# syghmon/bridges-with-reinforcement-learning

Hardware: AMD Instinct MI355X
Metric: env-steps/sec (vectorised assembly_gym, tower_height=4) (higher is better)
Workload: dtype f64

## Files before the change

bridges-with-reinforcement-learning_amd/bridges_hip/abi.py:

```python
import ctypes as C
import os

HERE = os.path.dirname(os.path.abspath(__file__))
LIB_PATH = os.environ.get("BRIDGES_LIB", os.path.join(HERE, "libbridges_hip.so"))
CSRC_DIR = os.path.join(os.path.dirname(HERE), "csrc")
INCLUDE_DIR = os.path.join(os.path.dirname(os.path.dirname(HERE)), "include")
STAMP_PREFIX = "BRIDGES_SRC_HASH="


def source_hash():
    import hashlib
    h = hashlib.sha256()
    for tag, d in (("csrc", CSRC_DIR), ("include", INCLUDE_DIR)):
        for name in sorted(os.listdir(d)):
            path = os.path.join(d, name)
            if os.path.isfile(path) and not name.startswith("."):
                h.update(f"{tag}/{name}\0".encode())
                with open(path, "rb") as fh:
                    h.update(fh.read())
                h.update(b"\0")
    return h.hexdigest()


def library_stamp(path=None):
# ... 127 lines not shown
def lib():
    global _lib
    if _lib is not None:
        return _lib
    if not os.path.exists(LIB_PATH):
        raise BridgesHipError(
            f"{LIB_PATH} not found: build it with `python __graft_entry__.py build` "
            "(hipcc --offload-arch=gfx950).  There is no CPU fallback.")
    L = C.CDLL(LIB_PATH)
    vp, i32, i64, f64, f32 = C.c_void_p, C.c_int32, C.c_int64, C.c_double, C.c_float
    try:
        L.bridges_source_hash.restype = C.c_char_p
        stamp = L.bridges_source_hash().decode()[len(STAMP_PREFIX):]
    except AttributeError:
        stamp = "missing"
    want = source_hash()
    if stamp != want:
        raise BridgesHipError(f"{LIB_PATH} is stale: it was built from other sources (stamp {stamp[:16]}, sources {want[:16]}); "
                              "rebuild it with `python __graft_entry__.py build`")
    L.bridges_last_error.restype = C.c_char_p
    L.bridges_device_count.restype = C.c_int
    sigs = {
        "bridges_env_create": [C.POINTER(Task), C.POINTER(EnvBuffers), C.POINTER(vp)],
        "bridges_env_destroy": [vp],
        "bridges_env_reset": [vp, vp],
        "bridges_env_step": [vp, vp],
        "bridges_env_select_random": [vp, vp],
        "bridges_env_lockstep_random": [vp, vp],
        "bridges_env_refresh": [vp, vp],
        "bridges_env_candidate_stability": [vp, vp],
        "bridges_gate_create": [C.POINTER(vp)],
        "bridges_gate_destroy": [vp],
        "bridges_env_set_gate": [vp, vp],
        "bridges_env_timing_begin": [vp, i32],
        "bridges_env_timing_end": [vp, C.POINTER(C.c_double), C.POINTER(i32)],
        "bridges_shapes_upload": [C.POINTER(Shape), i32, C.POINTER(vp)],
        "bridges_shapes_free": [vp],
        "bridges_place": [vp, i32, vp, vp, vp, vp, vp, vp, vp, vp],
        "bridges_create_block": [vp, i32, vp, vp, vp, vp, vp, vp, vp, vp, vp, vp, vp],
        "bridges_pose_block": [vp, i32, vp, vp, vp, vp],
        "bridges_face_frames": [vp, i32, vp, vp, vp, vp],
        "bridges_contains_points": [vp, i32, vp, i32, vp, vp, vp],
        "bridges_raster": [vp, i32, vp, vp, vp, vp, vp, vp, vp],
        "bridges_raster_sized": [vp, i32, vp, vp, vp, vp, i32, vp, vp, vp],
        "bridges_render_blocks": [vp, i32, vp, vp, vp, i32, vp, i32, vp, vp],
        "bridges_bits_or": [i32, vp, vp, vp, vp],
        "bridges_action_features": [vp, i32, vp, vp, vp, vp, i32, f64, f64, f64, f64, vp, vp, vp, vp, vp, vp, vp, vp],
        "bridges_bits_to_f32": [i32, vp, vp, vp],
        "bridges_bits_linear": [i32, vp, vp, vp, i32, vp, vp, vp, vp],
        "bridges_sigmoid_dot": [i32, vp, i64, vp, i32, vp, vp],
        "bridges_bits_dot": [i32, vp, vp, vp, vp, vp, vp],
        "bridges_head_sigmoid_dot": [i32, i32, i32, vp, i64, vp, vp, vp, vp, vp, i32, vp],
        "bridges_linear_backward_log": [i32, i32, i32, vp, vp, vp, vp, vp, vp, vp, vp, i64, vp, i32, vp, i32, vp, vp, vp],
        "bridges_mlp_mid_rows": [i32, i32, vp, vp, vp, vp, i64, vp, i64, vp, vp],
        "bridges_mlp_mid_supported": [i32, i32, vp],
        "bridges_mlp_mid_forward": [i32, i32, vp, vp, vp, vp, vp],
        "bridges_mlp_mid_backward": [i32, i32, vp, vp, vp, vp, vp, vp, vp, vp, vp, vp, i64, vp, f64, f64, f64, f64, vp],
        "bridges_eps_greedy_select": [i32, i32, vp, vp, vp, vp, vp, C.c_float, i32, vp, vp, vp, vp, vp, vp, vp, vp],
        "bridges_valid_rows": [i32, vp, vp, vp, vp, vp, vp, vp, vp, vp, vp, vp, vp],
        "bridges_env_groups": [i32, i32, vp, vp, vp, vp, vp, vp, vp, vp],
        "bridges_record_state": [i32, i32, vp, vp, vp, vp, vp, vp, vp, vp, vp, vp],
        "bridges_record_result": [i32, vp, vp, vp, vp, vp, vp],
        "bridges_replay_unpack": [i32, i32, i32, vp, vp, i32, i32, i32, i32, vp, vp, vp, vp, vp, vp, vp, vp, vp, vp, vp, vp],
        "bridges_bits_accumulate": [i32, vp, vp, vp, vp, vp, vp],
        "bridges_stability": [vp, i32, i32, vp, vp, vp, vp, vp, f64, f64, f64, f64, vp, vp, vp, i64, vp],
        "bridges_stability_penalty": [vp, i32, i32, vp, vp, vp, vp, vp, f64, f64, f64, f64, f64, vp, vp, vp, vp, i64, vp],
# ... 6 lines not shown
        "bridges_linear_forward": [i32, i32, i32, vp, vp, vp, i32, vp, vp, i64, vp, vp],
        "bridges_linear_backward": [i32, i32, i32, vp, vp, vp, vp, vp, vp, vp, vp, i64, vp, i32, vp],
        "bridges_mlp_input": [i32, i32, i32, i32, vp, vp, vp, vp, vp, vp, vp, vp],
        "bridges_mlp_input_batches": [i32, i32, i32, i32, i32, vp, vp, vp, vp, vp, vp, vp],
        "bridges_successor_loss": [i32, i32, i32, i32, vp, vp, vp, vp, vp, i32, i32, vp, vp, vp, vp, i32, vp, vp, vp, vp],
        "bridges_adam_step": [vp, vp, vp, vp, i64, vp, f64, f64, f64, f64, vp],
        "bridges_linear_backward_adam": [i32, i32, i32, vp, vp, vp, vp, vp, vp, vp, vp, vp, vp, vp, vp, i64, vp, f64, f64, f64, f64, vp, i32, vp],
        "bridges_conv3x3": [vp, vp, vp, vp, vp, vp, i64, i32, i32, i32, i32, i32, vp],
        "bridges_conv3x3_wgrad_scratch": [i64, i32, i32, i32, C.POINTER(i64)],
        "bridges_conv3x3_wgrad": [vp, vp, vp, vp, vp, vp, i64, i64, i32, i32, i32, vp],
        "bridges_maxpool2": [vp, vp, i64, i32, i32, vp],
        "bridges_bias_grad": [vp, vp, vp, i64, i64, i32, i32, vp],
        "bridges_adam_multi": [vp, i32, vp, vp, i32, vp, f64, f64, f64, f64, vp],
        "bridges_reduce_jobs": [vp, i32, i32, vp],
        "bridges_upconv2x2_backward_scratch": [i64, i32, i32, i32, i32, C.POINTER(i64)],
        "bridges_upconv2x2_backward": [vp, vp, vp, vp, vp, vp, vp, i64, i64, i32, i32, i32, i32, vp],
        "bridges_conv1x1_o1_forward": [vp, vp, vp, vp, i64, i32, i32, vp],
        "bridges_conv1x1_o1_backward": [vp, vp, vp, vp, vp, vp, vp, i64, i64, i32, i32, vp],
        "bridges_maxpool2_relu_backward": [vp, vp, vp, i64, i32, i32, vp],
        "bridges_td_target": [i32, vp, vp, vp, vp, i64, vp, vp, vp, f32, i32, vp, vp, vp, vp],
    }
    for name, argtypes in sigs.items():
        fn = getattr(L, name)
        fn.argtypes = argtypes
        fn.restype = C.c_int
    _lib = L
    return L


EXPORTED_SYMBOLS = (
    "bridges_last_error", "bridges_device_count", "bridges_source_hash", "bridges_env_create", "bridges_env_destroy",
    "bridges_env_reset", "bridges_env_step", "bridges_env_select_random", "bridges_env_lockstep_random", "bridges_env_refresh",
    "bridges_env_candidate_stability",
    "bridges_gate_create", "bridges_gate_destroy", "bridges_env_set_gate",
    "bridges_env_timing_begin", "bridges_env_timing_end",
    "bridges_place", "bridges_create_block", "bridges_pose_block", "bridges_face_frames", "bridges_contains_points", "bridges_raster", "bridges_raster_sized", "bridges_render_blocks", "bridges_action_features", "bridges_bits_or", "bridges_bits_to_f32", "bridges_bits_linear", "bridges_bits_dot", "bridges_bits_accumulate", "bridges_head_sigmoid_dot", "bridges_linear_backward_log", "bridges_mlp_mid_rows", "bridges_mlp_mid_supported", "bridges_mlp_mid_forward", "bridges_mlp_mid_backward", "bridges_eps_greedy_select", "bridges_valid_rows", "bridges_env_groups", "bridges_record_state", "bridges_record_result", "bridges_replay_unpack", "bridges_sigmoid_dot", "bridges_stability", "bridges_stability_penalty",
    "bridges_shapes_upload", "bridges_shapes_free", "bridges_soft_update", "bridges_td_target", "bridges_bias_relu", "bridges_bias_relu_pool2",
    "bridges_conv3x3_relu_o16", "bridges_conv3x3_relu_o16_ex", "bridges_conv3x3", "bridges_conv3x3_wgrad_scratch", "bridges_conv3x3_wgrad",
    "bridges_maxpool2", "bridges_maxpool2_relu_backward", "bridges_bias_grad", "bridges_adam_multi", "bridges_reduce_jobs", "bridges_upconv2x2_backward_scratch", "bridges_upconv2x2_backward", "bridges_conv1x1_o1_forward", "bridges_conv1x1_o1_backward", "bridges_upconv2x2", "bridges_linear_forward", "bridges_linear_backward", "bridges_mlp_input", "bridges_mlp_input_batches", "bridges_successor_loss", "bridges_adam_step", "bridges_linear_backward_adam",
)


def check(rc, what=""):
    if rc != 0:
        msg = lib().bridges_last_error().decode(errors="replace")
        raise BridgesHipError(f"{what} failed (rc={rc}): {msg}")


def require_gpu():
    import torch
    L = lib()
    if not torch.cuda.is_available() or L.bridges_device_count() <= 0:
        raise BridgesHipError("no MI355X / HIP device visible: the assembly_gym hot path runs only on the "
                              "HIP kernels of libbridges_hip.so (no CPU fallback)")
    return L


def current_stream():
    import torch
    return C.c_void_p(torch._C._cuda_getCurrentRawStream(torch._C._cuda_getDevice()))
```

bridges-with-reinforcement-learning_amd/csrc/api.hip:

```cpp
#include <hip/hip_runtime.h>
#include <cstdio>
#include <cstdlib>
#include <cstring>
#include <new>

#include "env_kernels.hip"
#include "ops_kernels.hip"
#include "dqn_kernels.hip"
#include "mlp_kernels.hip"
#include "conv_kernels.hip"
#include "conv_train_kernels.hip"

using namespace bridges;

static thread_local char g_err[512] = "";

static int fail_hip(hipError_t e, const char* what) {
    snprintf(g_err, sizeof(g_err), "%s: %s", what, hipGetErrorString(e));
    return BRIDGES_E_HIP;
}
static int fail_arg(const char* what) {
    snprintf(g_err, sizeof(g_err), "bad argument: %s", what);
    return BRIDGES_E_ARG;
}
#define HIP_TRY(x)                                        \
    do {                                                  \
        hipError_t e_ = (x);                              \
        if (e_ != hipSuccess) return fail_hip(e_, #x);    \
    } while (0)
#define LAUNCH_CHECK(name)                                       \
    do {                                                         \
        hipError_t e_ = hipGetLastError();                       \
        if (e_ != hipSuccess) return fail_hip(e_, name);         \
    } while (0)

struct bridges_gate {
    hipEvent_t last;
};

struct bridges_env {
    bridges_gate* gate;
    hipEvent_t raster_done;
    DevCtx ctx;
    TaskTable* tt_dev;
    int32_t* h_total;
    int max_blocks;
    int max_faces;
    hipEvent_t* ev_start;
    hipEvent_t* ev_stop;
    int ev_cap, ev_used;
};

extern "C" {

const char* bridges_last_error(void) { return g_err; }

#ifndef BRIDGES_SRC_HASH
#define BRIDGES_SRC_HASH "unstamped"
#endif
const char* bridges_source_hash(void) { return "BRIDGES_SRC_HASH=" BRIDGES_SRC_HASH; }

int bridges_device_count(void) {
    int n = 0;
    if (hipGetDeviceCount(&n) != hipSuccess) return 0;
    return n;
}

int bridges_env_create(const bridges_task* t, const bridges_env_buffers* buf, bridges_env** out) {
    if (!t || !buf || !out) return fail_arg("null");
    if (t->n_envs <= 0) return fail_arg("n_envs");
    if (t->max_blocks <= 0 || t->max_blocks > BRIDGES_MAX_BLOCKS) return fail_arg("max_blocks > BRIDGES_MAX_BLOCKS");
    if (t->n_shapes <= 0 || t->n_shapes > 8) return fail_arg("n_shapes");
    if (t->n_groups <= 0 || t->n_groups > BRIDGES_MAX_GROUPS) return fail_arg("n_groups");
    if (t->n_ground < 0 || t->n_ground > 32 || t->n_offsets <= 0 || t->n_offsets > 8) return fail_arg("n_ground/n_offsets");
    if (t->n_targets < 0 || t->n_targets > BRIDGES_MAX_TARGETS) return fail_arg("n_targets");
// ... 28 lines not shown
    memcpy(host->offsets, t->offsets, sizeof(double) * t->n_offsets);
    const int img = t->img_size ? t->img_size : IMG;
    for (int i = 0; i < IMG; ++i) {
        host->grid_x[i] = t->grid_x[i < img ? i : img - 1];
        host->grid_y[i] = t->grid_y[i < img ? i : img - 1];
    }
    hipError_t e = hipMalloc((void**)&env->tt_dev, sizeof(TaskTable));
    if (e == hipSuccess) e = hipMemcpy(env->tt_dev, host, sizeof(TaskTable), hipMemcpyHostToDevice);
    delete host;
    if (e != hipSuccess) { delete env; return fail_hip(e, "task table upload"); }
    DevCtx& c = env->ctx;
    memset(&c, 0, sizeof(c));
    c.b = *buf;
    c.tt = env->tt_dev;
    c.E = t->n_envs; c.K = t->max_blocks; c.max_steps = t->max_steps; c.a_max = t->a_max;
    c.n_groups = t->n_groups; c.n_ground = t->n_ground; c.n_offsets = t->n_offsets; c.n_targets = t->n_targets;
    memcpy(c.group_shape, t->group_shape, sizeof(c.group_shape));
    memcpy(c.group_face, t->group_face, sizeof(c.group_face));
    c.mu = t->mu; c.density = t->density; c.floor_hw = t->floor_half_width; c.floor_depth = t->floor_depth;
    c.xlim0 = t->xlim[0]; c.xlim1 = t->xlim[1]; c.ylim0 = t->ylim[0]; c.ylim1 = t->ylim[1];
    memcpy(c.targets, t->targets, sizeof(c.targets));
    c.seed = t->seed;
    c.debug = t->debug;
    c.env_id_base = t->env_id_base;
    c.n_shapes = t->n_shapes;
    c.img = img;
    hipDeviceProp_t prop;
    int dev = 0;
    (void)hipGetDevice(&dev);
    env->ev_start = env->ev_stop = nullptr;
    env->ev_cap = env->ev_used = 0;
    env->gate = nullptr;
    env->raster_done = nullptr;
    int cus = 256;
    if (hipGetDeviceProperties(&prop, dev) == hipSuccess && prop.multiProcessorCount > 0) cus = prop.multiProcessorCount;
    (void)cus;
    e = hipHostMalloc((void**)&env->h_total, sizeof(int32_t), hipHostMallocMapped | hipHostMallocCoherent);
    if (e == hipSuccess) e = hipHostGetDevicePointer((void**)&c.h_total, env->h_total, 0);
    if (e != hipSuccess) { (void)hipFree(env->tt_dev); delete env; return fail_hip(e, "hipHostMalloc"); }
    *env->h_total = t->n_envs * 64;
    env->max_blocks = 1 << 22;
    env->max_faces = 0;
    for (int g = 0; g < t->n_groups; ++g) {
        const int nv = t->shapes[t->group_shape[g]].nv;
        if (nv > env->max_faces) env->max_faces = nv;
    }
    *out = env;
    return BRIDGES_OK;
}

static void free_events(bridges_env* env) {
    for (int i = 0; i < env->ev_cap; ++i) {
        (void)hipEventDestroy(env->ev_start[i]);
        (void)hipEventDestroy(env->ev_stop[i]);
    }
    delete[] env->ev_start;
    delete[] env->ev_stop;
    env->ev_start = env->ev_stop = nullptr;
    env->ev_cap = env->ev_used = 0;
}

int bridges_env_destroy(bridges_env* env) {
    if (!env) return BRIDGES_OK;
    free_events(env);
    if (env->raster_done) (void)hipEventDestroy(env->raster_done);
    (void)hipFree(env->tt_dev);
    (void)hipHostFree(env->h_total);
    delete env;
    return BRIDGES_OK;
}

int bridges_gate_create(bridges_gate** out) {
    if (!out) return fail_arg("gate_create");
    bridges_gate* g = new (std::nothrow) bridges_gate();
    if (!g) return fail_arg("oom");
    g->last = nullptr;
    *out = g;
    return BRIDGES_OK;
}

int bridges_gate_destroy(bridges_gate* gate) {
    delete gate;
    return BRIDGES_OK;
}

int bridges_env_set_gate(bridges_env* env, bridges_gate* gate) {
    if (!env) return fail_arg("set_gate");
    if (gate && !env->raster_done) HIP_TRY(hipEventCreateWithFlags(&env->raster_done, hipEventDisableTiming));
    env->gate = gate;
    return BRIDGES_OK;
}

int bridges_env_timing_begin(bridges_env* env, int32_t max_launches) {
    if (!env || max_launches <= 0 || max_launches > (1 << 16)) return fail_arg("timing_begin");
    free_events(env);
    env->ev_start = new (std::nothrow) hipEvent_t[max_launches];
    env->ev_stop = new (std::nothrow) hipEvent_t[max_launches];
    if (!env->ev_start || !env->ev_stop) {
        delete[] env->ev_start;
        delete[] env->ev_stop;
        env->ev_start = env->ev_stop = nullptr;
        return fail_arg("oom");
    }
    for (int i = 0; i < max_launches; ++i) {
        HIP_TRY(hipEventCreate(&env->ev_start[i]));
        HIP_TRY(hipEventCreate(&env->ev_stop[i]));
        env->ev_cap = i + 1;
    }
    env->ev_used = 0;
    return BRIDGES_OK;
}

int bridges_env_timing_end(bridges_env* env, double* raster_ms_total, int32_t* n_launches) {
    if (!env || !raster_ms_total || !n_launches) return fail_arg("timing_end");
    double total = 0.0;
    for (int i = 0; i < env->ev_used; ++i) {
        HIP_TRY(hipEventSynchronize(env->ev_stop[i]));
        float ms = 0.f;
        HIP_TRY(hipEventElapsedTime(&ms, env->ev_start[i], env->ev_stop[i]));
        total += ms;
    }
    *raster_ms_total = total;
    *n_launches = env->ev_used;
    free_events(env);
    return BRIDGES_OK;
}

#ifndef RASTER_DYN_LDS
#define RASTER_DYN_LDS 0
#endif
static int refresh(bridges_env* env, hipStream_t s, int after_step) {
    const DevCtx& c = env->ctx;
    hipLaunchKernelGGL(k_scan, dim3(1), dim3(SCAN_THREADS), 0, s, c, after_step);
    LAUNCH_CHECK("k_scan");
    hipLaunchKernelGGL(k_enumerate, dim3(c.E), dim3(WAVE), 0, s, c);
    LAUNCH_CHECK("k_enumerate");
    long long est = (long long)(*(volatile int32_t*)env->h_total);
    if (est < c.E) est = c.E;
    est += est / 32 + 64;
    const long long items_est = est + c.E;
    long long rblocks = (items_est + 3) / 4;
    if (rblocks > env->max_blocks) rblocks = env->max_blocks;
    const bool timed = env->ev_cap > 0 && env->ev_used < env->ev_cap;
    if (env->gate && env->gate->last) HIP_TRY(hipStreamWaitEvent(s, env->gate->last, 0));
    if (timed) HIP_TRY(hipEventRecord(env->ev_start[env->ev_used], s));
    if (env->max_faces <= 4) hipLaunchKernelGGL(k_raster<4>, dim3((unsigned)rblocks), dim3(256), RASTER_DYN_LDS, s, c);
    else hipLaunchKernelGGL(k_raster<MAXV>, dim3((unsigned)rblocks), dim3(256), RASTER_DYN_LDS, s, c);
    LAUNCH_CHECK("k_raster");
    if (timed) { HIP_TRY(hipEventRecord(env->ev_stop[env->ev_used], s)); env->ev_used++; }
    if (env->gate) {
        HIP_TRY(hipEventRecord(env->raster_done, s));
        env->gate->last = env->raster_done;
    }
    hipLaunchKernelGGL(k_select, dim3(c.E), dim3(WAVE), 0, s, c, 0);
    LAUNCH_CHECK("k_select");
    return BRIDGES_OK;
}

int bridges_env_reset(bridges_env* env, void* stream) {
    if (!env) return fail_arg("null env");
    hipStream_t s = (hipStream_t)stream;
    hipLaunchKernelGGL(k_reset, dim3(env->ctx.E), dim3(WAVE), 0, s, env->ctx);
    LAUNCH_CHECK("k_reset");
    return refresh(env, s, 0);
}

int bridges_env_step(bridges_env* env, void* stream) {
    if (!env) return fail_arg("null env");
    hipStream_t s = (hipStream_t)stream;
    hipLaunchKernelGGL(k_step, dim3(env->ctx.E), dim3(WAVE), 0, s, env->ctx);
    LAUNCH_CHECK("k_step");
    return refresh(env, s, 1);
}

int bridges_env_refresh(bridges_env* env, void* stream) {
    if (!env) return fail_arg("null env");
    return refresh(env, (hipStream_t)stream, 0);
}

#ifndef CS_TAB_SMALL
#define CS_TAB_SMALL 768
#endif
#ifndef CS_COLS_SMALL
#define CS_COLS_SMALL 92
#endif
#define CS_TAB_LARGE 4096
int bridges_env_candidate_stability(bridges_env* env, void* stream) {
    if (!env) return fail_arg("null env");
    const DevCtx& c = env->ctx;
    if (!c.b.cand_stable || !c.b.cand_queue || !c.b.cand_counters || !c.b.cand_ws) return fail_arg("cand_stable / cand_queue / cand_counters / cand_ws not given");
    if (c.b.cand_ws_stride < (int64_t)(3 * c.K + 2) * (4 * BRIDGES_MAX_INTERFACES + 3)) return fail_arg("cand_ws_stride");
    hipStream_t s = (hipStream_t)stream;
    HIP_TRY(hipMemsetAsync(c.b.cand_counters, 0, 2 * sizeof(int32_t), s));
    long long est = (long long)(*(volatile int32_t*)env->h_total);
    if (est < c.E) est = c.E;
    est += est / 32 + 64;
    if (est > env->max_blocks) est = env->max_blocks;
    hipLaunchKernelGGL((k_candidate_stability<CS_TAB_SMALL, CS_COLS_SMALL, false>), dim3((unsigned)est), dim3(WAVE), 0, s, c);
    LAUNCH_CHECK("k_candidate_stability");
    const int drain = BRIDGES_CAND_WS_SLOTS;
    hipLaunchKernelGGL((k_candidate_stability<CS_TAB_LARGE, LP_MAX_COLS, true>), dim3(drain), dim3(WAVE), 0, s, c);
    LAUNCH_CHECK("k_candidate_stability (queue)");
    return BRIDGES_OK;
}

int bridges_env_select_random(bridges_env* env, void* stream) {
    if (!env) return fail_arg("null env");
    hipLaunchKernelGGL(k_select, dim3(env->ctx.E), dim3(WAVE), 0, (hipStream_t)stream, env->ctx, 1);
    LAUNCH_CHECK("k_select");
    return BRIDGES_OK;
}

int bridges_env_lockstep_random(bridges_env* env, void* stream) {
    int rc = bridges_env_select_random(env, stream);
    if (rc != BRIDGES_OK) return rc;
    return bridges_env_step(env, stream);
}

int bridges_shapes_upload(const bridges_shape* host, int32_t n, bridges_shape** out_dev) {
    if (!host || n <= 0 || !out_dev) return fail_arg("shapes_upload");
    HIP_TRY(hipMalloc((void**)out_dev, sizeof(bridges_shape) * n));
    HIP_TRY(hipMemcpy(*out_dev, host, sizeof(bridges_shape) * n, hipMemcpyHostToDevice));
    return BRIDGES_OK;
}

int bridges_shapes_free(bridges_shape* dev) {
    if (dev) HIP_TRY(hipFree(dev));
    return BRIDGES_OK;
}

int bridges_place(const bridges_shape* shapes_dev, int32_t n, const double* frame1, const int32_t* shape_id,
                  const int32_t* face, const double* ox, const double* oy, double* pose, double* verts, void* stream) {
    if (n < 0 || !shapes_dev) return fail_arg("bridges_place");
    if (n == 0) return BRIDGES_OK;
    hipLaunchKernelGGL(k_place, dim3((n + 255) / 256), dim3(256), 0, (hipStream_t)stream, shapes_dev, n, frame1,
                       shape_id, face, ox, oy, pose, verts);
    LAUNCH_CHECK("k_place");
    return BRIDGES_OK;
}

int bridges_create_block(const bridges_shape* shapes_dev, int32_t n, const double* target_verts,
                         const int32_t* target_shape, const int32_t* target_face, const int32_t* shape_id,
                         const int32_t* face, const double* ox, const double* oy, double* pose, double* verts,
                         double* target_frame_out, void* stream) {
    if (n < 0 || !shapes_dev) return fail_arg("bridges_create_block");
    if (n == 0) return BRIDGES_OK;
    hipLaunchKernelGGL(k_create_block, dim3((n + 255) / 256), dim3(256), 0, (hipStream_t)stream, shapes_dev, n,
                       target_verts, target_shape, target_face, shape_id, face, ox, oy, pose, verts, target_frame_out);
    LAUNCH_CHECK("k_create_block");
// ... 855 lines not shown
```

bridges-with-reinforcement-learning_amd/csrc/env_kernels.hip:

```cpp
#include "bridges_device.h"
#include "rbe_device.h"

namespace bridges {

__device__ inline void reset_env(const DevCtx& c, int e, int lane) {
    c.b.state_bits[(size_t)e * IMG + lane] = 0ull;
    if (lane < c.K) c.b.blk_occ[(size_t)e * c.K + lane] = 0;
    if (lane == 0) {
        c.b.n_blocks[e] = 0;
        c.b.n_if[e] = 0;
        c.b.targets_left[e] = (c.n_targets >= 32) ? 0xffffffffu : ((1u << c.n_targets) - 1u);
        c.b.needs_reset[e] = 0;
    }
}

__device__ inline int count_candidates(const DevCtx& c, int e, int nb, int lane) {
    int nfree = 0;
    for (int i0 = 0; i0 < nb * MAXV; i0 += WAVE) {
        int i = i0 + lane;
        bool fr = false;
        if (i < nb * MAXV) {
            int b = i / MAXV, f = i % MAXV;
            int nv = c.tt->shapes[c.b.blk_shape[(size_t)e * c.K + b]].nv;
            fr = f < nv && !((c.b.blk_occ[(size_t)e * c.K + b] >> f) & 1);
        }
        nfree += __popcll(__ballot(fr));
    }
    return c.n_groups * (c.n_ground + nfree * c.n_offsets);
}

__global__ __launch_bounds__(WAVE) void k_reset(DevCtx c) {
    int e = blockIdx.x, lane = threadIdx.x;
    reset_env(c, e, lane);
    if (lane < 8) c.b.step_flags[(size_t)e * 8 + lane] = 0;
    int nc = count_candidates(c, e, 0, lane);
    if (lane == 0) {
        c.b.reward[e] = 0.f;
        c.b.lin_reward[e] = 0.f;
        c.b.n_reached[e] = 0;
        c.b.draw_counter[e] = 0;
        c.b.n_cand[e] = nc;
    }
}

#define STEP_IF_LDS 32
#define STEP_TAB_LDS 4096
struct StepStage {
    bridges_shape shapes[8];
    double pose[MAXK * 4];
    double verts[MAXK * MAXV * 2];
    int32_t shape_id[MAXK];
    int32_t occ[MAXK];
};
struct StepKeep {
    double if_geom[STEP_IF_LDS * 8];
    int32_t if_body[STEP_IF_LDS * 2];
    double cen[MAXK * 2];
    double vol[MAXK];
};
static_assert(sizeof(StepStage) <= STEP_TAB_LDS * sizeof(double), "staging area must fit into the tableau storage");

__global__ __launch_bounds__(WAVE) void k_step(DevCtx c) {
    __shared__ __attribute__((aligned(16))) double tab[STEP_TAB_LDS];
    __shared__ LpScratch S;
    __shared__ StepKeep Lk;
    StepStage& L = *reinterpret_cast<StepStage*>(tab);
    __builtin_amdgcn_s_setprio(3);
    const int e = blockIdx.x, lane = threadIdx.x;
    const int K = c.K;
    uint8_t* flags = c.b.step_flags + (size_t)e * 8;
    const long long ts0 = DIAG(c, 8) ? wall_clock64() : 0;
    int32_t* shape_id_g = c.b.blk_shape + (size_t)e * K;
    double* pose_g = c.b.blk_pose + (size_t)e * K * 4;
    double* verts_g = c.b.blk_verts + (size_t)e * K * MAXV * 2;
    uint8_t* occ_g = c.b.blk_occ + (size_t)e * K;
    int32_t* if_body_g = c.b.if_body + (size_t)e * MAXIF * 2;
    double* if_geom_g = c.b.if_geom + (size_t)e * MAXIF * 8;
    double* ws = c.b.lp_ws + (size_t)e * c.b.lp_ws_stride;
    const WarmHdr* hdr_g = reinterpret_cast<const WarmHdr*>(ws);

    const uint8_t need_reset = c.b.needs_reset[e];
    const int a = c.b.sel_index[e];
    const int off = c.b.cand_offset[e];
    const int nb = c.b.n_blocks[e];
    const int n_if_old = c.b.n_if[e];
    uint32_t left = c.b.targets_left[e];
    const uint64_t sbits = c.b.state_bits[(size_t)e * IMG + lane];
    WarmPre W;
    W.magic = hdr_g->magic; W.n_blocks = hdr_g->n_blocks; W.n_if = hdr_g->n_if; W.stride = hdr_g->stride;
    W.half = hdr_g->half; W.m = hdr_g->m;
    W.basis_lane = hdr_g->basis[lane];
    {
        const double* src = reinterpret_cast<const double*>(c.tt->shapes);
        double* dst = reinterpret_cast<double*>(L.shapes);
        const int nd = c.n_shapes * (int)(sizeof(bridges_shape) / 8);
        for (int i = lane; i < nd; i += WAVE) dst[i] = src[i];
        for (int i = lane; i < nb * 4; i += WAVE) L.pose[i] = pose_g[i];
        for (int i = lane; i < nb * MAXV * 2; i += WAVE) L.verts[i] = verts_g[i];
        if (lane < K) { L.shape_id[lane] = shape_id_g[lane]; L.occ[lane] = occ_g[lane]; }
        const int n0 = n_if_old < STEP_IF_LDS ? n_if_old : STEP_IF_LDS;
        for (int i = lane; i < n0 * 8; i += WAVE) Lk.if_geom[i] = if_geom_g[i];
        for (int i = lane; i < n0 * 2; i += WAVE) Lk.if_body[i] = if_body_g[i];
    }

    if (need_reset) {
        reset_env(c, e, lane);
        if (lane < 8) flags[lane] = 0;
        if (lane == 0) {
            c.b.reward[e] = 0.f;
            c.b.lin_reward[e] = 0.f;
            c.b.n_reached[e] = 0;
        }
        if (lane == 0) c.b.n_cand[e] = c.n_groups * c.n_ground;
        return;
    }
// ... 224 lines not shown
            if (i < c.E) c.b.cand_offset[i] = carry + wbase + incl - v[u];
            __syncthreads();
            if (t == SCAN_THREADS - 1) carry_s = carry + wbase + incl;
            __syncthreads();
        }
    }
#pragma unroll
    for (int k = 0; k < 8; ++k) {
        unsigned long long x = acc[k];
#pragma unroll
        for (int o = 32; o > 0; o >>= 1) x += __shfl_xor(x, o, WAVE);
        if (lane == 0) red[wv][k] = x;
    }
    __syncthreads();
    if (t == 0) {
        unsigned long long tot[8] = {0, 0, 0, 0, 0, 0, 0, 0};
        for (int w = 0; w < SCAN_WAVES; ++w)
            for (int k = 0; k < 8; ++k) tot[k] += red[w][k];
        c.b.cand_offset[c.E] = carry_s;
        if (c.h_total) *c.h_total = carry_s;
        c.b.stats[ST_SUM_CAND] += (uint64_t)carry_s;
        c.b.stats[ST_SUM_BLOCKS] += tot[0];
        c.b.stats[ST_ENV_STEPS] += tot[1];
        c.b.stats[ST_RESET_ONLY] += tot[2];
        c.b.stats[ST_LP_ERRORS] += tot[3];
        c.b.stats[ST_IF_OVERFLOW] += tot[4];
        c.b.stats[ST_SUM_VALID] += tot[5];
        c.b.stats[ST_WARM_RESOLVED] += tot[6];
        c.b.stats[ST_CAND_OVERFLOW] += tot[7];
        c.b.stats[ST_LOCKSTEPS] += 1;
    }
}

__global__ __launch_bounds__(WAVE) void k_enumerate(DevCtx c) {
    __shared__ uint8_t free_b[MAXK * MAXV], free_f[MAXK * MAXV];
    __shared__ bridges_shape sh_l[8];
    __shared__ double verts_l[MAXK * MAXV * 2];
    __shared__ int32_t shape_l[MAXK], occ_l[MAXK];
    __shared__ double xg_l[32], offs_l[8];
    __builtin_amdgcn_s_setprio(3);
    const int e = blockIdx.x, lane = threadIdx.x;
    const int K = c.K;
    if (lane < 32) xg_l[lane] = c.tt->x_ground[lane];
    if (lane < 8) offs_l[lane] = c.tt->offsets[lane];
    const int nb = c.b.n_blocks[e];
    const int ncand = c.b.n_cand[e];
    const size_t off = (size_t)c.b.cand_offset[e];
    {
        const double* src = reinterpret_cast<const double*>(c.tt->shapes);
        double* dst = reinterpret_cast<double*>(sh_l);
        const int nd = c.n_shapes * (int)(sizeof(bridges_shape) / 8);
        for (int i = lane; i < nd; i += WAVE) dst[i] = src[i];
        const double* vg = c.b.blk_verts + (size_t)e * K * MAXV * 2;
        for (int i = lane; i < nb * MAXV * 2; i += WAVE) verts_l[i] = vg[i];
        if (lane < K) { shape_l[lane] = c.b.blk_shape[(size_t)e * K + lane]; occ_l[lane] = c.b.blk_occ[(size_t)e * K + lane]; }
    }
    __syncthreads();
    const bridges_shape* shapes = sh_l;
    const int32_t* shape_id = shape_l;
    const double* verts = verts_l;
    int nfree = 0;
    for (int i0 = 0; i0 < nb * MAXV; i0 += WAVE) {
        int i = i0 + lane;
        bool fr = false;
        int b = i / MAXV, f = i % MAXV;
        if (i < nb * MAXV) {
            int nv = shapes[shape_id[b]].nv;
            fr = f < nv && !((occ_l[b] >> f) & 1);
        }
        uint64_t bal = __ballot(fr);
        if (fr) {
            int idx = nfree + __popcll(bal & ((1ull << lane) - 1ull));
            free_b[idx] = (uint8_t)b;
            free_f[idx] = (uint8_t)f;
        }
        nfree += __popcll(bal);
    }
    __syncthreads();
    const int gsize = c.n_ground + nfree * c.n_offsets;
    for (int a = lane; a < ncand; a += WAVE) {
// ... 192 lines not shown
            const bool inb = (meta >> 24) & 1;
            (void)nv;
            double fr0 = 0.0, fr1 = 0.0, fr2 = 0.0, fr3 = 0.0;
            if (lane < MAXV) {
                const double2* p = reinterpret_cast<const double2*>(c.b.cand_frames + (ci * MAXV + lane) * 4);
                const double2 a = p[0], b = p[1];
                fr0 = a.x; fr1 = a.y; fr2 = b.x; fr3 = b.y;
            }
            const uint64_t occ = c.b.state_bits[(size_t)e * IMG + lane] | obst;
            uint64_t bits = 0ull;
            if (!DIAG(c, 2)) bits = (NF == 4 || nv <= 4) ? raster_rows<4>(fr0, fr1, fr2, fr3, c.img, X, Y, lane)
                                                         : raster_rows6(fr0, fr1, fr2, fr3, c.img, X, Y, lane);
            const bool overlap = __ballot((bits & occ) != 0ull) != 0ull;
            double p_hi, p_lo;
            raster_reward_fetch(bits, c.b.reward_prefix, lane, p_hi, p_lo);
            c.b.cand_bits[ci * IMG + lane] = bits;
            if (c.b.cand_raster && !DIAG(c, 4))
                write_f32_image(c.b.cand_raster + ci * IMG * IMG, bits, lane, c.b.cand_raster_nz ? c.b.cand_raster_nz + ci : nullptr);
            const double lin = raster_reward_sum(p_hi, p_lo);
            if (lane == 0) {
                c.b.cand_lin[ci] = (float)lin;
                c.b.cand_mask[ci] = (uint8_t)(inb && !overlap);
            }
        } else {
            const int e = it - total;
            write_f32_image(c.b.state_raster + (size_t)e * IMG * IMG, c.b.state_bits[(size_t)e * IMG + lane], lane,
                            c.b.state_raster_nz ? c.b.state_raster_nz + e : nullptr);
        }
    }
}

__global__ __launch_bounds__(WAVE) void k_select(DevCtx c, int draw) {
    const int e = blockIdx.x, lane = threadIdx.x;
    const int nc = c.b.n_cand[e];
    const size_t off = (size_t)c.b.cand_offset[e];
    int nvalid = 0;
    for (int a0 = 0; a0 < nc; a0 += WAVE) {
        int a = a0 + lane;
        nvalid += __popcll(__ballot(a < nc && c.b.cand_mask[off + a]));
    }
    int sel = 0;
    if (nvalid > 0 && draw) {
        uint64_t ctr = c.b.draw_counter[e];
        uint64_t r = splitmix64(splitmix64(((c.seed & 0xFFFFFFFFull) << 32) | (uint32_t)(c.env_id_base + e)) ^ ctr);
        int rank = (int)(r % (uint64_t)nvalid);
        int seen = 0;
        for (int a0 = 0; a0 < nc; a0 += WAVE) {
            int a = a0 + lane;
            uint64_t bal = __ballot(a < nc && c.b.cand_mask[off + a]);
            int cnt = __popcll(bal);
            if (rank < seen + cnt) {
                int want = rank - seen;
                for (int k = 0; k < want; ++k) bal &= bal - 1;
                sel = a0 + (__ffsll((long long)bal) - 1);
                break;
            }
            seen += cnt;
        }
    }
    if (lane == 0) {
        if (draw) {
            c.b.sel_index[e] = sel;
            if (nvalid > 0) c.b.draw_counter[e] += 1;
        } else {
            c.b.n_valid[e] = nvalid;
            if (nvalid == 0) {
                c.b.needs_reset[e] = 1;
                c.b.step_flags[(size_t)e * 8 + F_NO_ACTIONS] = 1;
            }
        }
    }
}

#ifndef CS_NEW_IF
#define CS_NEW_IF 16
#endif
#ifndef CS_WAVES
#define CS_WAVES 4
#endif
template <int TAB, int MAXCOLS, bool QUEUE>
__global__ __launch_bounds__(WAVE) __attribute__((amdgpu_waves_per_eu(QUEUE ? 1 : CS_WAVES, QUEUE ? 2 : CS_WAVES))) void k_candidate_stability(DevCtx c) {
    __shared__ __attribute__((aligned(16))) double tab[TAB];
    __shared__ LpScratchT<MAXCOLS> S;
    __shared__ double new_geom[CS_NEW_IF * 8];
    __shared__ int32_t new_body[CS_NEW_IF * 2];
    const int lane = threadIdx.x;
    const int K = c.K;
    const bridges_shape* shapes = c.tt->shapes;
    const int total = c.b.cand_offset[c.E];
    int32_t* cnt = c.b.cand_counters;
    const int qlen = QUEUE ? cnt[0] : 0;
    for (int item = blockIdx.x;; item += gridDim.x) {
        int ci;
        if constexpr (QUEUE) {
            int i = 0;
            if (lane == 0) i = atomicAdd(&cnt[1], 1);
            i = __builtin_amdgcn_readfirstlane(i);
            if (i >= qlen) return;
            ci = c.b.cand_queue[i];
        } else {
            if (item >= total) return;
            ci = item;
// ... 112 lines not shown
```

include/bridges_hip.h:

```cpp
#ifndef BRIDGES_HIP_H
#define BRIDGES_HIP_H

#include <stdint.h>

#ifdef __cplusplus
extern "C" {
#endif

#define BRIDGES_OK 0
#define BRIDGES_E_ARG (-1)
#define BRIDGES_E_HIP (-2)
#define BRIDGES_E_NODEV (-3)

#define BRIDGES_MAX_VERTS 6
#define BRIDGES_MAX_BLOCKS 16
#define BRIDGES_MAX_GROUPS 24
#define BRIDGES_MAX_TARGETS 8
#define BRIDGES_MAX_INTERFACES 64
#define BRIDGES_IMG 64
#define BRIDGES_LP_WS_DOUBLES (64 + 2 * (3 * BRIDGES_MAX_BLOCKS + 2) * (4 * BRIDGES_MAX_INTERFACES + 2 + 3 * BRIDGES_MAX_BLOCKS + 1))
#define BRIDGES_LP_SNAP_DOUBLES (64 + (3 * BRIDGES_MAX_BLOCKS + 2) * (4 * BRIDGES_MAX_INTERFACES + 2 + 3 * BRIDGES_MAX_BLOCKS + 1))
#define BRIDGES_CAND_WS_SLOTS 1024

typedef struct {
// ... 75 lines not shown
    const uint64_t* obstacle_bits;
    const float* reward_map;
    const double* reward_prefix;
    double* lp_ws;
    int64_t lp_ws_stride;
    uint64_t* stats;
    uint8_t* cand_stable;
    int32_t* cand_queue;
    int32_t* cand_counters;
    double* cand_ws;
    int64_t cand_ws_stride;
    double* lp_snap;
    int64_t lp_snap_stride;
} bridges_env_buffers;

typedef struct bridges_env bridges_env;

const char* bridges_last_error(void);
int bridges_device_count(void);
const char* bridges_source_hash(void);

int bridges_env_create(const bridges_task* task, const bridges_env_buffers* buf, bridges_env** out);
int bridges_env_destroy(bridges_env* env);
int bridges_env_reset(bridges_env* env, void* stream);
int bridges_env_step(bridges_env* env, void* stream);
int bridges_env_select_random(bridges_env* env, void* stream);
int bridges_env_lockstep_random(bridges_env* env, void* stream);
int bridges_env_timing_begin(bridges_env* env, int32_t max_launches);
int bridges_env_timing_end(bridges_env* env, double* raster_ms_total, int32_t* n_launches);
typedef struct bridges_gate bridges_gate;
int bridges_gate_create(bridges_gate** out);
int bridges_gate_destroy(bridges_gate* gate);
int bridges_env_set_gate(bridges_env* env, bridges_gate* gate);
int bridges_env_refresh(bridges_env* env, void* stream);
int bridges_env_candidate_stability(bridges_env* env, void* stream);

int bridges_place(const bridges_shape* shapes_dev, int32_t n, const double* frame1, const int32_t* shape_id,
                  const int32_t* face, const double* ox, const double* oy, double* pose, double* verts,
                  void* stream);
int bridges_create_block(const bridges_shape* shapes_dev, int32_t n, const double* target_verts,
                         const int32_t* target_shape, const int32_t* target_face, const int32_t* shape_id,
                         const int32_t* face, const double* ox, const double* oy, double* pose, double* verts,
                         double* target_frame_out, void* stream);
int bridges_pose_block(const bridges_shape* shapes_dev, int32_t n, const int32_t* shape_id, const double* pose,
                       double* verts, void* stream);
int bridges_face_frames(const bridges_shape* shapes_dev, int32_t n, const int32_t* shape_id, const double* verts,
                        double* frames, void* stream);
int bridges_contains_points(const bridges_shape* shapes_dev, int32_t shape_id, const double* verts, int32_t n,
                            const double* points, uint8_t* inside, void* stream);
int bridges_raster(const bridges_shape* shapes_dev, int32_t n, const double* verts, const int32_t* shape_id,
                   const double* grid_x, const double* grid_y, uint64_t* bits, float* img, void* stream);
int bridges_render_blocks(const bridges_shape* shapes_dev, int32_t n, const double* verts, const int32_t* shape_id,
                          const double* grid_x, int32_t W, const double* grid_y, int32_t H, uint8_t* out, void* stream);
int bridges_raster_sized(const bridges_shape* shapes_dev, int32_t n, const double* verts, const int32_t* shape_id,
                         const double* grid_x, const double* grid_y, int32_t size, uint64_t* bits, float* img,
                         void* stream);
int bridges_action_features(const bridges_shape* shapes_dev, int32_t n, const double* verts, const int32_t* shape_id,
                            const double* grid_x, const double* grid_y, int32_t size, double xlim0, double xlim1, double ylim0,
                            double ylim1, const uint64_t* state_bits, const uint64_t* obstacle_bits, const double* reward_prefix,
                            uint64_t* bits, float* img, uint8_t* mask, float* lin_reward, void* stream);
int bridges_bits_or(int32_t n_groups, const int32_t* ranges, const uint64_t* bits, uint64_t* out, void* stream);
int bridges_bits_to_f32(int32_t n, const uint64_t* bits, float* img, void* stream);
int bridges_bits_linear(int32_t n_rows, const uint64_t* bits, const int64_t* bits_row, const float* wt, int32_t d,
                        const float* base, const int64_t* base_row, float* out, void* stream);
int bridges_bits_dot(int32_t n_rows, const uint64_t* bits, const int64_t* bits_row, const float* img, const int64_t* slot,
                     float* out, void* stream);
// ... 140 lines not shown
```

Baseline: 4.936 million.

## Fuse candidate prefix scan into enumerate and random draw into step kernel

For small environment counts, each k_enumerate block now computes its own candidate offset by reducing the n_cand array with vectorised loads. A separate k_stats kernel runs after enumerate for the statistics, which removes the serialised k_scan launch that previously came before enumerate. Lockstep random stepping now draws the action inside k_step instead of launching k_select first, which saves one launch per step. The trade-off is that every enumerate block re-reads the whole n_cand prefix. The change also adds a candidate_hint API and reuses timing events for the gate.

```diff
diff --git a/bridges-with-reinforcement-learning_amd/bridges_hip/abi.py b/bridges-with-reinforcement-learning_amd/bridges_hip/abi.py
--- a/bridges-with-reinforcement-learning_amd/bridges_hip/abi.py
+++ b/bridges-with-reinforcement-learning_amd/bridges_hip/abi.py
@@ -183,6 +183,7 @@
         "bridges_gate_create": [C.POINTER(vp)],
         "bridges_gate_destroy": [vp],
         "bridges_env_set_gate": [vp, vp],
+        "bridges_env_candidate_hint": [vp, C.POINTER(i32)],
         "bridges_env_timing_begin": [vp, i32],
         "bridges_env_timing_end": [vp, C.POINTER(C.c_double), C.POINTER(i32)],
         "bridges_shapes_upload": [C.POINTER(Shape), i32, C.POINTER(vp)],
@@ -255,7 +256,7 @@
     "bridges_last_error", "bridges_device_count", "bridges_source_hash", "bridges_env_create", "bridges_env_destroy",
     "bridges_env_reset", "bridges_env_step", "bridges_env_select_random", "bridges_env_lockstep_random", "bridges_env_refresh",
     "bridges_env_candidate_stability",
-    "bridges_gate_create", "bridges_gate_destroy", "bridges_env_set_gate",
+    "bridges_gate_create", "bridges_gate_destroy", "bridges_env_set_gate", "bridges_env_candidate_hint",
     "bridges_env_timing_begin", "bridges_env_timing_end",
     "bridges_place", "bridges_create_block", "bridges_pose_block", "bridges_face_frames", "bridges_contains_points", "bridges_raster", "bridges_raster_sized", "bridges_render_blocks", "bridges_action_features", "bridges_bits_or", "bridges_bits_to_f32", "bridges_bits_linear", "bridges_bits_dot", "bridges_bits_accumulate", "bridges_head_sigmoid_dot", "bridges_linear_backward_log", "bridges_mlp_mid_rows", "bridges_mlp_mid_supported", "bridges_mlp_mid_forward", "bridges_mlp_mid_backward", "bridges_eps_greedy_select", "bridges_valid_rows", "bridges_env_groups", "bridges_record_state", "bridges_record_result", "bridges_replay_unpack", "bridges_sigmoid_dot", "bridges_stability", "bridges_stability_penalty",
     "bridges_shapes_upload", "bridges_shapes_free", "bridges_soft_update", "bridges_td_target", "bridges_bias_relu", "bridges_bias_relu_pool2",
diff --git a/bridges-with-reinforcement-learning_amd/csrc/api.hip b/bridges-with-reinforcement-learning_amd/csrc/api.hip
--- a/bridges-with-reinforcement-learning_amd/csrc/api.hip
+++ b/bridges-with-reinforcement-learning_amd/csrc/api.hip
@@ -41,6 +41,7 @@
 struct bridges_env {
     bridges_gate* gate;
     hipEvent_t raster_done;
+    bool fused_scan;
     DevCtx ctx;
     TaskTable* tt_dev;
     int32_t* h_total;
@@ -135,6 +136,7 @@
     env->ev_cap = env->ev_used = 0;
     env->gate = nullptr;
     env->raster_done = nullptr;
+    env->fused_scan = t->n_envs <= FUSED_SCAN_MAX_E && ((uintptr_t)buf->n_cand & 15) == 0;
     int cus = 256;
     if (hipGetDeviceProperties(&prop, dev) == hipSuccess && prop.multiProcessorCount > 0) cus = prop.multiProcessorCount;
     (void)cus;
@@ -154,6 +156,10 @@
 
 static void free_events(bridges_env* env) {
     for (int i = 0; i < env->ev_cap; ++i) {
+        if (env->gate && env->gate->last == env->ev_stop[i]) {
+            (void)hipEventSynchronize(env->ev_stop[i]);
+            env->gate->last = nullptr;
+        }
         (void)hipEventDestroy(env->ev_start[i]);
         (void)hipEventDestroy(env->ev_stop[i]);
     }
@@ -191,6 +197,12 @@
     if (!env) return fail_arg("set_gate");
     if (gate && !env->raster_done) HIP_TRY(hipEventCreateWithFlags(&env->raster_done, hipEventDisableTiming));
     env->gate = gate;
+    return BRIDGES_OK;
+}
+
+int bridges_env_candidate_hint(bridges_env* env, int32_t* out) {
+    if (!env || !out) return fail_arg("candidate_hint");
+    *out = *(volatile int32_t*)env->h_total;
     return BRIDGES_OK;
 }
 
@@ -234,10 +246,18 @@
 #endif
 static int refresh(bridges_env* env, hipStream_t s, int after_step) {
     const DevCtx& c = env->ctx;
-    hipLaunchKernelGGL(k_scan, dim3(1), dim3(SCAN_THREADS), 0, s, c, after_step);
-    LAUNCH_CHECK("k_scan");
-    hipLaunchKernelGGL(k_enumerate, dim3(c.E), dim3(WAVE), 0, s, c);
-    LAUNCH_CHECK("k_enumerate");
+    const bool fused = after_step && env->fused_scan;
+    if (fused) {
+        hipLaunchKernelGGL(k_enumerate<true>, dim3(c.E), dim3(WAVE), 0, s, c);
+        LAUNCH_CHECK("k_enumerate");
+        hipLaunchKernelGGL(k_stats, dim3(1), dim3(SCAN_THREADS), 0, s, c);
+        LAUNCH_CHECK("k_stats");
+    } else {
+        hipLaunchKernelGGL(k_scan, dim3(1), dim3(SCAN_THREADS), 0, s, c, after_step);
+        LAUNCH_CHECK("k_scan");
+        hipLaunchKernelGGL(k_enumerate<false>, dim3(c.E), dim3(WAVE), 0, s, c);
+        LAUNCH_CHECK("k_enumerate");
+    }
     long long est = (long long)(*(volatile int32_t*)env->h_total);
     if (est < c.E) est = c.E;
     est += est / 32 + 64;
@@ -250,11 +270,16 @@
     if (env->max_faces <= 4) hipLaunchKernelGGL(k_raster<4>, dim3((unsigned)rblocks), dim3(256), RASTER_DYN_LDS, s, c);
     else hipLaunchKernelGGL(k_raster<MAXV>, dim3((unsigned)rblocks), dim3(256), RASTER_DYN_LDS, s, c);
     LAUNCH_CHECK("k_raster");
-    if (timed) { HIP_TRY(hipEventRecord(env->ev_stop[env->ev_used], s)); env->ev_used++; }
+    if (timed) HIP_TRY(hipEventRecord(env->ev_stop[env->ev_used], s));
     if (env->gate) {
-        HIP_TRY(hipEventRecord(env->raster_done, s));
-        env->gate->last = env->raster_done;
-    }
+        if (timed) {
+            env->gate->last = env->ev_stop[env->ev_used];
+        } else {
+            HIP_TRY(hipEventRecord(env->raster_done, s));
+            env->gate->last = env->raster_done;
+        }
+    }
+    if (timed) env->ev_used++;
     hipLaunchKernelGGL(k_select, dim3(c.E), dim3(WAVE), 0, s, c, 0);
     LAUNCH_CHECK("k_select");
     return BRIDGES_OK;
@@ -268,12 +293,16 @@
     return refresh(env, s, 0);
 }
 
+static int step(bridges_env* env, hipStream_t s, bool draw) {
+    if (draw) hipLaunchKernelGGL(k_step<true>, dim3(env->ctx.E), dim3(WAVE), 0, s, env->ctx);
+    else hipLaunchKernelGGL(k_step<false>, dim3(env->ctx.E), dim3(WAVE), 0, s, env->ctx);
+    LAUNCH_CHECK("k_step");
+    return refresh(env, s, 1);
+}
+
 int bridges_env_step(bridges_env* env, void* stream) {
     if (!env) return fail_arg("null env");
-    hipStream_t s = (hipStream_t)stream;
-    hipLaunchKernelGGL(k_step, dim3(env->ctx.E), dim3(WAVE), 0, s, env->ctx);
-    LAUNCH_CHECK("k_step");
-    return refresh(env, s, 1);
+    return step(env, (hipStream_t)stream, false);
 }
 
 int bridges_env_refresh(bridges_env* env, void* stream) {
@@ -315,9 +344,8 @@
 }
 
 int bridges_env_lockstep_random(bridges_env* env, void* stream) {
-    int rc = bridges_env_select_random(env, stream);
-    if (rc != BRIDGES_OK) return rc;
-    return bridges_env_step(env, stream);
+    if (!env) return fail_arg("null env");
+    return step(env, (hipStream_t)stream, true);
 }
 
 int bridges_shapes_upload(const bridges_shape* host, int32_t n, bridges_shape** out_dev) {
diff --git a/bridges-with-reinforcement-learning_amd/csrc/env_kernels.hip b/bridges-with-reinforcement-learning_amd/csrc/env_kernels.hip
--- a/bridges-with-reinforcement-learning_amd/csrc/env_kernels.hip
+++ b/bridges-with-reinforcement-learning_amd/csrc/env_kernels.hip
@@ -41,6 +41,45 @@
         c.b.draw_counter[e] = 0;
         c.b.n_cand[e] = nc;
     }
+}
+
+__device__ inline int count_valid(const DevCtx& c, int nc, size_t off, int lane) {
+    int nvalid = 0;
+    for (int a0 = 0; a0 < nc; a0 += WAVE) {
+        int a = a0 + lane;
+        nvalid += __popcll(__ballot(a < nc && c.b.cand_mask[off + a]));
+    }
+    return nvalid;
+}
+
+__device__ inline int select_random(const DevCtx& c, int e, int lane) {
+    const int nc = c.b.n_cand[e];
+    const size_t off = (size_t)c.b.cand_offset[e];
+    const int nvalid = count_valid(c, nc, off, lane);
+    int sel = 0;
+    if (nvalid > 0) {
+        uint64_t ctr = c.b.draw_counter[e];
+        uint64_t r = splitmix64(splitmix64(((c.seed & 0xFFFFFFFFull) << 32) | (uint32_t)(c.env_id_base + e)) ^ ctr);
+        int rank = (int)(r % (uint64_t)nvalid);
+        int seen = 0;
+        for (int a0 = 0; a0 < nc; a0 += WAVE) {
+            int a = a0 + lane;
+            uint64_t bal = __ballot(a < nc && c.b.cand_mask[off + a]);
+            int cnt = __popcll(bal);
+            if (rank < seen + cnt) {
+                int want = rank - seen;
+                for (int k = 0; k < want; ++k) bal &= bal - 1;
+                sel = a0 + (__ffsll((long long)bal) - 1);
+                break;
+            }
+            seen += cnt;
+        }
+    }
+    if (lane == 0) {
+        c.b.sel_index[e] = sel;
+        if (nvalid > 0) c.b.draw_counter[e] += 1;
+    }
+    return sel;
 }
 
 #define STEP_IF_LDS 32
@@ -60,6 +99,7 @@
 };
 static_assert(sizeof(StepStage) <= STEP_TAB_LDS * sizeof(double), "staging area must fit into the tableau storage");
 
+template <bool DRAW>
 __global__ __launch_bounds__(WAVE) void k_step(DevCtx c) {
     __shared__ __attribute__((aligned(16))) double tab[STEP_TAB_LDS];
     __shared__ LpScratch S;
@@ -80,7 +120,7 @@
     const WarmHdr* hdr_g = reinterpret_cast<const WarmHdr*>(ws);
 
     const uint8_t need_reset = c.b.needs_reset[e];
-    const int a = c.b.sel_index[e];
+    const int a = DRAW ? select_random(c, e, lane) : c.b.sel_index[e];
     const int off = c.b.cand_offset[e];
     const int nb = c.b.n_blocks[e];
     const int n_if_old = c.b.n_if[e];
@@ -371,6 +411,85 @@
     }
 }
 
+__global__ __launch_bounds__(SCAN_THREADS) void k_stats(DevCtx c) {
+    __shared__ unsigned long long red[SCAN_WAVES][8];
+    const int t = threadIdx.x, lane = t & 63, wv = t >> 6;
+    unsigned long long acc[8] = {0, 0, 0, 0, 0, 0, 0, 0};
+    for (int base0 = 0; base0 < c.E; base0 += SCAN_THREADS * SCAN_BATCH) {
+        int nbk[SCAN_BATCH], nval[SCAN_BATCH];
+        uint64_t fl8[SCAN_BATCH];
+#pragma unroll
+        for (int u = 0; u < SCAN_BATCH; ++u) {
+            const int i = base0 + u * SCAN_THREADS + t;
+            const bool in = i < c.E;
+            nbk[u] = in ? c.b.n_blocks[i] : 0;
+            nval[u] = in ? c.b.n_valid[i] : 0;
+            fl8[u] = in ? *reinterpret_cast<const uint64_t*>(c.b.step_flags + (size_t)i * 8) : 0ull;
+        }
+#pragma unroll
+        for (int u = 0; u < SCAN_BATCH; ++u) {
+            if (base0 + u * SCAN_THREADS + t >= c.E) continue;
+            const unsigned valid = (unsigned)(fl8[u] >> (8 * F_VALID)) & 0xffu;
+            const unsigned lperr = (unsigned)(fl8[u] >> (8 * F_LP_ERROR)) & 0xffu;
+            acc[0] += (unsigned long long)nbk[u];
+            acc[1] += valid ? 1 : 0;
+            acc[2] += valid ? 0 : 1;
+            acc[3] += (lperr & 1) ? 1 : 0;
+            acc[4] += (lperr & 2) ? 1 : 0;
+            acc[5] += (unsigned long long)nval[u];
+            acc[6] += (lperr & 4) ? 1 : 0;
+            acc[7] += (lperr & 8) ? 1 : 0;
+        }
+    }
+#pragma unroll
+    for (int k = 0; k < 8; ++k) {
+        unsigned long long x = acc[k];
+#pragma unroll
+        for (int o = 32; o > 0; o >>= 1) x += __shfl_xor(x, o, WAVE);
+        if (lane == 0) red[wv][k] = x;
+    }
+    __syncthreads();
+    if (t == 0) {
+        unsigned long long tot[8] = {0, 0, 0, 0, 0, 0, 0, 0};
+        for (int w = 0; w < SCAN_WAVES; ++w)
+            for (int k = 0; k < 8; ++k) tot[k] += red[w][k];
+        c.b.stats[ST_SUM_CAND] += (uint64_t)c.b.cand_offset[c.E];
+        c.b.stats[ST_SUM_BLOCKS] += tot[0];
+        c.b.stats[ST_ENV_STEPS] += tot[1];
+        c.b.stats[ST_RESET_ONLY] += tot[2];
+        c.b.stats[ST_LP_ERRORS] += tot[3];
+        c.b.stats[ST_IF_OVERFLOW] += tot[4];
+        c.b.stats[ST_SUM_VALID] += tot[5];
+        c.b.stats[ST_WARM_RESOLVED] += tot[6];
+        c.b.stats[ST_CAND_OVERFLOW] += tot[7];
+        c.b.stats[ST_LOCKSTEPS] += 1;
+    }
+}
+
+#define FUSED_SCAN_MAX_E (4 * WAVE * SCAN_BATCH * 4)
+
+__device__ __forceinline__ int cand_prefix(const DevCtx& c, int e, int lane) {
+    const int4* n4 = reinterpret_cast<const int4*>(c.b.n_cand);
+    const int quads = e >> 2;
+    const int am = c.a_max;
+    const int ti = (quads << 2) + lane;
+    int s = lane < (e & 3) ? min(c.b.n_cand[ti], am) : 0;
+    for (int q0 = 0; q0 < quads; q0 += WAVE * SCAN_BATCH) {
+        int4 v[SCAN_BATCH];
+#pragma unroll
+        for (int u = 0; u < SCAN_BATCH; ++u) {
+            const int q = q0 + u * WAVE + lane;
+            v[u] = q < quads ? n4[q] : make_int4(0, 0, 0, 0);
+        }
+#pragma unroll
+        for (int u = 0; u < SCAN_BATCH; ++u) s += min(v[u].x, am) + min(v[u].y, am) + min(v[u].z, am) + min(v[u].w, am);
+    }
+#pragma unroll
+    for (int o = 32; o > 0; o >>= 1) s += __shfl_xor(s, o, WAVE);
+    return s;
+}
+
+template <bool FUSED>
 __global__ __launch_bounds__(WAVE) void k_enumerate(DevCtx c) {
     __shared__ uint8_t free_b[MAXK * MAXV], free_f[MAXK * MAXV];
     __shared__ bridges_shape sh_l[8];
@@ -383,8 +502,28 @@
     if (lane < 32) xg_l[lane] = c.tt->x_ground[lane];
     if (lane < 8) offs_l[lane] = c.tt->offsets[lane];
     const int nb = c.b.n_blocks[e];
-    const int ncand = c.b.n_cand[e];
-    const size_t off = (size_t)c.b.cand_offset[e];
+    int ncand = c.b.n_cand[e];
+    size_t off;
+    if (FUSED) {
+        const int pre = cand_prefix(c, e, lane);
+        if (ncand > c.a_max) {
+            ncand = c.a_max;
+            if (lane == 0) {
+                c.b.n_cand[e] = ncand;
+                c.b.step_flags[(size_t)e * 8 + F_LP_ERROR] |= 8;
+            }
+        }
+        off = (size_t)pre;
+        if (lane == 0) {
+            c.b.cand_offset[e] = pre;
+            if (e == c.E - 1) {
+                c.b.cand_offset[c.E] = pre + ncand;
+                if (c.h_total) *c.h_total = pre + ncand;
+            }
+        }
+    } else {
+        off = (size_t)c.b.cand_offset[e];
+    }
     {
         const double* src = reinterpret_cast<const double*>(c.tt->shapes);
         double* dst = reinterpret_cast<double*>(sh_l);
@@ -643,42 +782,16 @@
 
 __global__ __launch_bounds__(WAVE) void k_select(DevCtx c, int draw) {
     const int e = blockIdx.x, lane = threadIdx.x;
-    const int nc = c.b.n_cand[e];
-    const size_t off = (size_t)c.b.cand_offset[e];
-    int nvalid = 0;
-    for (int a0 = 0; a0 < nc; a0 += WAVE) {
-        int a = a0 + lane;
-        nvalid += __popcll(__ballot(a < nc && c.b.cand_mask[off + a]));
-    }
-    int sel = 0;
-    if (nvalid > 0 && draw) {
-        uint64_t ctr = c.b.draw_counter[e];
-        uint64_t r = splitmix64(splitmix64(((c.seed & 0xFFFFFFFFull) << 32) | (uint32_t)(c.env_id_base + e)) ^ ctr);
-        int rank = (int)(r % (uint64_t)nvalid);
-        int seen = 0;
-        for (int a0 = 0; a0 < nc; a0 += WAVE) {
-            int a = a0 + lane;
-            uint64_t bal = __ballot(a < nc && c.b.cand_mask[off + a]);
-            int cnt = __popcll(bal);
-            if (rank < seen + cnt) {
-                int want = rank - seen;
-                for (int k = 0; k < want; ++k) bal &= bal - 1;
-                sel = a0 + (__ffsll((long long)bal) - 1);
-                break;
-            }
-            seen += cnt;
-        }
-    }
+    if (draw) {
+        select_random(c, e, lane);
+        return;
+    }
+    const int nvalid = count_valid(c, c.b.n_cand[e], (size_t)c.b.cand_offset[e], lane);
     if (lane == 0) {
-        if (draw) {
-            c.b.sel_index[e] = sel;
-            if (nvalid > 0) c.b.draw_counter[e] += 1;
-        } else {
-            c.b.n_valid[e] = nvalid;
-            if (nvalid == 0) {
-                c.b.needs_reset[e] = 1;
-                c.b.step_flags[(size_t)e * 8 + F_NO_ACTIONS] = 1;
-            }
+        c.b.n_valid[e] = nvalid;
+        if (nvalid == 0) {
+            c.b.needs_reset[e] = 1;
+            c.b.step_flags[(size_t)e * 8 + F_NO_ACTIONS] = 1;
         }
     }
 }
diff --git a/include/bridges_hip.h b/include/bridges_hip.h
--- a/include/bridges_hip.h
+++ b/include/bridges_hip.h
@@ -131,6 +131,7 @@
 int bridges_gate_create(bridges_gate** out);
 int bridges_gate_destroy(bridges_gate* gate);
 int bridges_env_set_gate(bridges_env* env, bridges_gate* gate);
+int bridges_env_candidate_hint(bridges_env* env, int32_t* out);
 int bridges_env_refresh(bridges_env* env, void* stream);
 int bridges_env_candidate_stability(bridges_env* env, void* stream);
 
```

After: 5.030 million, median of 6. 1.02x the previous value.
